# Tom-Ryder/VIforSDEs

Measured on AMD Instinct MI355X. Metric: sampled-paths/sec + ELBO-iters/sec (value = global_batch * ELBO-iters/s), higher is better.
Workload: dtype f32 (GRU/ELBO kernels) + bf16-autocast encoder; 1 GPU; lv: state_dim=2, T=400 (dt=0.1), batch=512/GPU, enc 256x8x4 heads, GRU 64x2; global_batch=512, parallelism=dp1, hip_graph=True

## Files before the change

### include/vsde_hip.h

```cpp
#ifndef VSDE_HIP_H
#define VSDE_HIP_H

#include <stddef.h>
#include <stdint.h>

#ifdef __cplusplus
extern "C" {
#endif

#define VSDE_ABI_VERSION 1

#define VSDE_E_BADARG (-1)
#define VSDE_E_LAYERS (-2)
#define VSDE_E_HIDDEN (-3)
#define VSDE_E_WORKSPACE (-4)
#define VSDE_E_STATE (-5)

#define VSDE_MAX_LAYERS 4
#define VSDE_MAX_HIDDEN 1024
#define VSDE_MAX_STATE 32

#define VSDE_CTX_F32 0
#define VSDE_CTX_BF16 1

// ... 83 lines not shown
                            int N, int C, int64_t mod_pitch, void *workspace, size_t workspace_bytes, void *stream);
int vsde_swiglu_fwd(int dtype, const void *u, void *out, int64_t M, int H2, void *stream);
int vsde_swiglu_bwd(int dtype, const void *u, const void *dout, void *du, int64_t M, int H2, void *stream);
int vsde_gate_merge_fwd(int dtype, const void *attn, const void *glog, void *out, int64_t B, int N, int heads, int d,
                        int token_major, int64_t glog_stride, void *stream);
int vsde_gate_merge_bwd(int dtype, const void *attn, const void *glog, const void *dout, void *dattn, void *dglog, int64_t B,
                        int N, int heads, int d, int token_major, int64_t glog_stride, void *stream);
int vsde_qk_norm_rope_fwd(int dtype, const void *qkv, const float *cosT, const float *sinT, const float *wq, const float *wk,
                          const void *v0, const float *lam, void *q, void *k, void *v, int64_t B, int N, int heads, int d,
                          double eps, int token_major, int64_t row_stride, void *stream);
int64_t vsde_qk_norm_rope_bwd_partials(int64_t B, int N, int heads, int d);
int vsde_qk_norm_rope_bwd(int dtype, const void *qkv, const float *cosT, const float *sinT, const float *wq, const float *wk,
                          const void *v0, const float *lam, const void *dq, const void *dk, const void *dv, void *dqkv,
                          void *dv0, float *dlam_partial, int64_t B, int N, int heads, int d, double eps, int token_major,
                          int64_t row_stride, int dv0_accumulate, const void *dv_extra, void *stream);

int vsde_attention_max_tokens(void);
int vsde_attention_fwd_bf16(const void *q, const void *k, const void *v, void *o, float *lse, int64_t B, int N, int H,
                            int head_dim, double scale, void *stream);
int vsde_attention_bwd_bf16(const void *dout, const void *q, const void *k, const void *v, const void *o, const float *lse,
                            void *dq, void *dk, void *dv, float *delta, int64_t B, int N, int H, int head_dim, double scale,
                            void *stream);

int vsde_attention_fused_supported(int N, int head_dim);
int vsde_attention_fwd_gated_bf16(const void *q, const void *k, const void *v, const void *gate, int64_t ldg, void *o, float *lse,
                                  int64_t B, int N, int H, double scale, void *stream);
int vsde_gate_bwd_delta(const void *dout, const void *og, const void *gate, int64_t ldg, void *dattn, void *dgate, int64_t ldd,
                        float *delta, int64_t B, int N, int H, void *stream);
int64_t vsde_attention_bwd_fused_partials(int64_t B, int N, int H);
int vsde_attention_bwd_fused_bf16(const void *dattn, const void *q, const void *k, const void *v, const float *lse, const float *delta,
                                  const float *rinv, const float *cosT, const float *sinT, const float *wq, const float *wk,
                                  const void *vdiff, const float *lam, void *dv0, int dv0_accumulate, const void *dv_extra, void *dy,
                                  int64_t ldy, float *dlam_partial, int64_t B, int N, int H, double scale, void *stream);

size_t vsde_linear_wgrad_workspace_bytes(int64_t M, int N, int K);
int vsde_linear_wgrad_bf16(const void *dy, const void *x, int64_t M, int N, int K, float *dW, float *db, void *workspace,
                           size_t workspace_bytes, void *stream);
int vsde_linear_wgrad_bf16_rows(const void *dy, const void *x, int64_t M, int N, int K, float *dW, float *db,
                                const int32_t *row_map, void *workspace, size_t workspace_bytes, void *stream);
typedef struct VsdeWgradItem {
    const void *dy, *x;
    int64_t M;
    int32_t N, K;
    float *dW, *db;
    const int32_t *row_map;
} VsdeWgradItem;
size_t vsde_linear_wgrad_group_workspace_bytes(int n, const void *items );
int vsde_linear_wgrad_group_bf16(int n, const void *items, int group_plan, void *workspace, size_t workspace_bytes, void *stream);

#define VSDE_EPI_PLAIN 0
#define VSDE_EPI_SWIGLU 1
#define VSDE_EPI_SWIGLU_BWD 2
int vsde_linear_bf16_supported(int64_t M, int N, int K, int epilogue);
int vsde_linear_bf16(const void *x, int64_t ldx, const void *w, const void *bias, void *y, int64_t ldy, int64_t M, int N, int K,
                     int epilogue, void *s_out, int64_t lds, const void *u_in, int64_t ldu, void *stream);
int vsde_linear_qknorm_bf16(const void *x, int64_t ldx, const void *w, const void *bias, int64_t M, int K, int heads, int gate_width,
                            int tokens, const float *cosT, const float *sinT, const float *wq, const float *wk, const void *v0,
                            const float *lam, double eps, void *q, void *k, void *v, void *gate, int64_t ldg, int gate_sigmoid,
                            float *rinv, void *vdiff, void *stream);
int vsde_linear_gated_bf16(const void *attn, int64_t ldx, const void *gate, int64_t ldgate, const void *w, const void *bias, void *y,
                           int64_t ldy, int64_t M, int N, int K, void *stream);

int vsde_linear_gate_bwd_bf16(const void *dy, int64_t ldy, const void *w_t, const void *og, const void *s, int64_t lds, void *dattn,
                              void *dgate, int64_t ldd, float *delta, int64_t M, int K, int heads, int tokens, void *stream);

int vsde_mlp_block_fwd_bf16(const void *x, const void *yin, const void *ga, const void *sc, const void *sh, const void *gm,
// ... 69 lines not shown
```

### viforsdes_amd/_hip.py

```python
from __future__ import annotations

import ctypes
import os
from typing import Optional, Sequence

import torch

from .build import LIB_PATH

VSDE_ABI_VERSION = 1
MAX_LAYERS = 4
MAX_HIDDEN = 1024
MAX_STATE = 32
DIAG_MIN = 1e-2


class HipLibraryError(RuntimeError):
    pass


class _Dims(ctypes.Structure):
    _fields_ = [(n, ctypes.c_int) for n in ("B", "T", "S", "P", "C", "H", "L")]


class _Weights(ctypes.Structure):
    _fields_ = [(n, ctypes.c_void_p) for n in (
        "W_ih_l0", "W_hh_l0", "b_ih_l0", "b_hh_l0", "W_ih_stack", "W_hh_stack",
        "b_ih_stack", "b_hh_stack", "out_weight", "out_bias")]


class _CtxView(ctypes.Structure):
    _fields_ = [("base", ctypes.c_void_p), ("dtype", ctypes.c_int),
                ("batch_stride", ctypes.c_int64), ("step_stride", ctypes.c_int64)]


class _Grads(ctypes.Structure):
    _fields_ = [(n, ctypes.c_void_p) for n in (
        "x0", "context", "theta", "W_ih_l0", "W_hh_l0", "b_ih_l0", "b_hh_l0",
        "W_ih_stack", "W_hh_stack", "b_ih_stack", "b_hh_stack", "out_weight", "out_bias")] + [
        ("context_dtype", ctypes.c_int), ("context_batch_stride", ctypes.c_int64)]


EXPORTS = (
    "vsde_abi_version", "vsde_build_ablations", "vsde_last_error",
    "vsde_head_forward_workspace_bytes", "vsde_head_forward",
    "vsde_head_backward_workspace_bytes", "vsde_head_backward",
    "vsde_elbo_path_terms", "vsde_elbo_path_terms_bwd", "vsde_elbo_tail_fwd", "vsde_elbo_tail_bwd",
    "vsde_log_weights", "vsde_log_weight_accumulate",
    "vsde_profile_enable", "vsde_profile_elapsed_ms", "vsde_debug_force_v1", "vsde_debug_head_mp", "vsde_head_mfma_range_exceeded",
    "vsde_ln_modulate_fwd", "vsde_ln_modulate_bwd", "vsde_gated_residual_fwd", "vsde_gated_residual_bwd",
    "vsde_swiglu_fwd", "vsde_swiglu_bwd", "vsde_gate_merge_fwd", "vsde_gate_merge_bwd",
    "vsde_qk_norm_rope_fwd", "vsde_qk_norm_rope_bwd_partials", "vsde_qk_norm_rope_bwd",
    "vsde_residual_ln_fwd", "vsde_residual_ln_bwd", "vsde_colsum_workspace_bytes", "vsde_linear_wgrad_workspace_bytes", "vsde_linear_wgrad_bf16", "vsde_linear_wgrad_bf16_rows", "vsde_linear_wgrad_group_workspace_bytes", "vsde_linear_wgrad_group_bf16",
    "vsde_attention_max_tokens", "vsde_attention_fwd_bf16", "vsde_attention_bwd_bf16",
    "vsde_attention_fused_supported", "vsde_attention_fwd_gated_bf16", "vsde_gate_bwd_delta", "vsde_attention_bwd_fused_partials",
    "vsde_attention_bwd_fused_bf16",
    "vsde_euler_maruyama_fwd", "vsde_euler_maruyama_bwd", "vsde_sde_coefficients_fwd", "vsde_sde_coefficients_bwd", "vsde_linear_bf16_supported", "vsde_linear_bf16", "vsde_linear_qknorm_bf16", "vsde_linear_gated_bf16", "vsde_linear_gate_bwd_bf16",
    "vsde_mlp_image_bytes", "vsde_mlp_fwd_bf16", "vsde_mlp_block_fwd_bf16", "vsde_mlp_attn_block_fwd_bf16", "vsde_linear_deep256_bf16", "vsde_mlp_debug_trace", "vsde_wgrad_debug_trace", "vsde_attn_debug_trace", "vsde_mlp_bwd_image_bytes", "vsde_mlp_bwd_bf16",
    "vsde_pack_tile_bytes", "vsde_pack_refresh", "vsde_optim_chunk_bytes", "vsde_optim_chunk_elems", "vsde_optim_step",
)

_lib: Optional[ctypes.CDLL] = None
_loaded_path: Optional[str] = None


def library_path() -> str:
    return _loaded_path or os.environ.get("VSDE_HIP_LIB") or LIB_PATH


def has_ablations() -> bool:
    return bool(load().vsde_build_ablations())


ABL_LIB_PATH = os.path.join(os.path.dirname(LIB_PATH), "libvsde_hip_abl.so")


def load() -> ctypes.CDLL:
    global _lib
    if _lib is not None:
        return _lib
    path = os.environ.get("VSDE_HIP_LIB") or LIB_PATH
    if not os.path.exists(path):
        raise HipLibraryError(
            f"{path} is missing: build it with `python -m viforsdes_amd.build` "
            "(there is no CPU fallback for the fused head / ELBO kernels)")
    lib = ctypes.CDLL(path)
    for name in EXPORTS:
        if not hasattr(lib, name):
            raise HipLibraryError(f"{path} does not export {name}")
    global _loaded_path
    _loaded_path = path
    lib.vsde_abi_version.restype = ctypes.c_int
    if lib.vsde_abi_version() != VSDE_ABI_VERSION:
        raise HipLibraryError(f"{path}: ABI version mismatch; rebuild it")
    lib.vsde_last_error.restype = ctypes.c_char_p
    lib.vsde_head_forward_workspace_bytes.restype = ctypes.c_size_t
    lib.vsde_head_backward_workspace_bytes.restype = ctypes.c_size_t
    for f in (lib.vsde_head_forward, lib.vsde_head_backward, lib.vsde_elbo_path_terms, lib.vsde_elbo_path_terms_bwd):
        f.restype = ctypes.c_int
    lib.vsde_qk_norm_rope_bwd_partials.restype = ctypes.c_int64
    lib.vsde_attention_bwd_fused_partials.restype = ctypes.c_int64
    lib.vsde_linear_wgrad_workspace_bytes.restype = ctypes.c_size_t
    lib.vsde_linear_wgrad_group_workspace_bytes.restype = ctypes.c_size_t
    lib.vsde_colsum_workspace_bytes.restype = ctypes.c_size_t
    lib.vsde_mlp_bwd_image_bytes.restype = ctypes.c_int64
    _lib = lib
    return lib


def _raise(rc: int) -> None:
    msg = load().vsde_last_error().decode("utf-8", "replace")
    if rc < 0:
        raise ValueError(msg)
    raise HipLibraryError(f"HIP error {rc}: {msg}")


def _ptr(t: Optional[torch.Tensor]):
    return ctypes.c_void_p(None if t is None or t.numel() == 0 else t.data_ptr())


def _require_hip(*tensors: torch.Tensor) -> torch.device:
    dev = None
    for t in tensors:
        if t is None:
            continue
        if not t.is_cuda:
            raise HipLibraryError(
                "the fused head / ELBO kernels only run on a HIP (cuda) device; got a "
                f"{t.device} tensor and there is no CPU fallback")
        if dev is None:
            dev = t.device
        elif t.device != dev:
            raise ValueError("all tensors must live on the same device")
    assert dev is not None
# ... 803 lines not shown
    du = torch.empty(M, 2 * H, device=dev, dtype=torch.bfloat16)
    dx = torch.empty(M, C, device=dev, dtype=torch.bfloat16)
    with torch.cuda.device(dev):
        _call(lib.vsde_mlp_bwd_bf16, _ptr(dy), _i64(lddy), _ptr(u), _i64(ldu), _ptr(img), _ptr(du), _i64(2 * H), _ptr(dx), _i64(C), _i64(M),
              ctypes.c_int(C), ctypes.c_int(H), _stream(dev))
    return du, dx


def linear_gate_bwd(dy: torch.Tensor, w_t: torch.Tensor, og: torch.Tensor, s: torch.Tensor, dgate: torch.Tensor, tokens: int):
    lib = load(); dev = _require_hip(dy, w_t, og, s, dgate)
    dy, ldy = _rows2d(dy); s, lds = _rows2d(s); dgate, ldd = _rows2d(dgate)
    B, N, H, d = og.shape
    M, K = dy.shape
    if d != 64 or N != tokens or M != B * N or tuple(w_t.shape) != (H * 64, K) or not (og.is_contiguous() and w_t.is_contiguous()):
        raise ValueError("linear_gate_bwd: inconsistent shapes")
    dattn = torch.empty_like(og)
    delta = torch.empty(B, H, N, device=dev, dtype=torch.float32)
    with torch.cuda.device(dev):
        _call(lib.vsde_linear_gate_bwd_bf16, _ptr(dy), _i64(ldy), _ptr(w_t), _ptr(og), _ptr(s), _i64(lds), _ptr(dattn), _ptr(dgate),
              _i64(ldd), _ptr(delta), _i64(M), ctypes.c_int(K), ctypes.c_int(H), ctypes.c_int(N), _stream(dev))
    return dattn, delta


def attention_bwd_fused(dattn, q, k, v, lse, delta, rinv, cos, sin, wq, wk, vdiff, lam, dv0, dv_extra, dy, scale: float):
    lib = load(); dev = _require_hip(dattn, q, k, v, lse, delta, rinv, dy)
    B, N, H, d = q.shape
    dy2, ldy = _rows2d(dy)
    accumulate = dv0 is not None
    parts = None
    if vdiff is not None:
        if dv0 is None:
            dv0 = torch.empty_like(v)
        parts = torch.empty(int(lib.vsde_attention_bwd_fused_partials(_i64(B), ctypes.c_int(N), ctypes.c_int(H))), device=dev, dtype=torch.float32)
    with torch.cuda.device(dev):
        _call(lib.vsde_attention_bwd_fused_bf16, _ptr(dattn), _ptr(q), _ptr(k), _ptr(v), _ptr(lse), _ptr(delta), _ptr(rinv), _ptr(cos),
              _ptr(sin), _ptr(wq), _ptr(wk), _ptr(vdiff), _ptr(lam if vdiff is not None else None),
              _ptr(dv0 if vdiff is not None else None), ctypes.c_int(int(accumulate)), _ptr(dv_extra), _ptr(dy2), _i64(ldy), _ptr(parts),
              _i64(B), ctypes.c_int(N), ctypes.c_int(H), ctypes.c_double(scale), _stream(dev))
    return (dv0 if vdiff is not None else None), (parts.sum() if parts is not None else None)


def linear_gated_bf16(attn: torch.Tensor, gate: torch.Tensor, w: torch.Tensor, bias: Optional[torch.Tensor]):
    lib = load(); dev = _require_hip(attn, gate, w)
    attn, ldx = _rows2d(attn); gate, ldg = _rows2d(gate)
    M, K = attn.shape
    N = w.shape[0]
    y = torch.empty(M, N, device=dev, dtype=torch.bfloat16)
    with torch.cuda.device(dev):
        _call(lib.vsde_linear_gated_bf16, _ptr(attn), _i64(ldx), _ptr(gate), _i64(ldg), _ptr(w), _ptr(bias), _ptr(y), _i64(N), _i64(M),
              ctypes.c_int(N), ctypes.c_int(K), _stream(dev))
    return y


def linear_swiglu_bwd_bf16(dy: torch.Tensor, w_t: torch.Tensor, u: torch.Tensor):
    lib = load(); dev = _require_hip(dy, w_t, u)
    dy, ldx = _rows2d(dy)
    M, K = dy.shape
    H = w_t.shape[0]
    du = torch.empty(M, 2 * H, device=dev, dtype=torch.bfloat16)
    with torch.cuda.device(dev):
        _call(lib.vsde_linear_bf16, _ptr(dy), _i64(ldx), _ptr(w_t), None, _ptr(du), _i64(2 * H), _i64(M), ctypes.c_int(H),
              ctypes.c_int(K), ctypes.c_int(EPI_SWIGLU_BWD), None, _i64(0), _ptr(u), _i64(u.stride(0)), _stream(dev))
    return du
```

### viforsdes_amd/csrc/vsde_attn.hip

```cpp
#include <stdlib.h>

#include "vsde_common.h"

namespace vsde {

typedef float f32x16 __attribute__((ext_vector_type(16)));
typedef short bf16x8 __attribute__((ext_vector_type(8)));
typedef short bf16x4 __attribute__((ext_vector_type(4)));
typedef __bf16 bf16v2 __attribute__((ext_vector_type(2)));
typedef float f32v2 __attribute__((ext_vector_type(2)));

constexpr int AT_D = 64;
constexpr int AT_KLD = 72;
constexpr int AT_MAXN = 544;

struct AttnParams {
    const uint16_t *q, *k, *v;
    uint16_t *o;
    float *lse;
    int N, H;
    int npad;
    int vld;
    float scale, scale_log2e;
    const uint16_t *gate;
// ... 592 lines not shown
            p.trace[wave * 8 + 7] = npairs_;
        }
    }
#undef VSDE_F8_STAMP
}
#endif


struct QkBwd {
    uint16_t *dy; int64_t ldy;
    const float *rinv;
    const float *cosT, *sinT;
    const float *wq, *wk;
    const float *lam;
    const uint16_t *vdiff;
    uint16_t *dv0; int dv0_accumulate;
    const uint16_t *dv_extra;
    float *dlam_partial;
    int dbg;
};

struct AttnBwdParams {
    const uint16_t *q, *k, *v, *o, *dout;
    const float *lse;
    float *delta;
    uint16_t *dq, *dk, *dv;
    int N, H, ntile;
    float scale, scale_log2e;
    QkBwd f;
    int park_off;
    int split_dq, split_dkv;
    int split_pitch_dq, split_pitch_dkv;
    int nragged;
};

__device__ __forceinline__ f32x16 tile_product(const uint16_t *arow, const bf16x8 (&bfrag)[4]) {
    f32x16 t = {0, 0, 0, 0, 0, 0, 0, 0, 0, 0, 0, 0, 0, 0, 0, 0};
#pragma unroll
    for (int ks = 0; ks < 4; ++ks) t = __builtin_amdgcn_mfma_f32_32x32x16_bf16(*(const bf16x8 *)(arow + ks * 16), bfrag[ks], t, 0, 0, 0);
    return t;
}

typedef short bf16x4s __attribute__((ext_vector_type(4)));
__device__ __forceinline__ uint2 lds_read_tr(const uint16_t *ptr) {
    bf16x4s r = __builtin_amdgcn_ds_read_tr16_b64_v4i16((__attribute__((address_space(3))) bf16x4s *)ptr);
    return *(uint2 *)&r;
}

__device__ __forceinline__ void accumulate_transposed(const uint16_t *tile, int lane, const bf16x8 &b0, const bf16x8 &b1,
                                                      f32x16 &acc0, f32x16 &acc1) {
    const int h2 = lane >> 5, m = lane & 15;
    const uint16_t *src = tile + (4 * h2 + (m >> 2)) * AT_KLD + ((lane >> 4) & 1) * 16 + (m & 3) * 4;
#pragma unroll
    for (int dt = 0; dt < 2; ++dt) {
        const uint2 a0 = lds_read_tr(src + dt * 32), a1 = lds_read_tr(src + dt * 32 + 8 * AT_KLD);
        const uint2 a2 = lds_read_tr(src + dt * 32 + 16 * AT_KLD), a3 = lds_read_tr(src + dt * 32 + 24 * AT_KLD);
        uint4 w0 = make_uint4(a0.x, a0.y, a1.x, a1.y), w1 = make_uint4(a2.x, a2.y, a3.x, a3.y);
        if (dt == 0) {
            acc0 = __builtin_amdgcn_mfma_f32_32x32x16_bf16(*(bf16x8 *)&w0, b0, acc0, 0, 0, 0);
            acc0 = __builtin_amdgcn_mfma_f32_32x32x16_bf16(*(bf16x8 *)&w1, b1, acc0, 0, 0, 0);
        } else {
            acc1 = __builtin_amdgcn_mfma_f32_32x32x16_bf16(*(bf16x8 *)&w0, b0, acc1, 0, 0, 0);
            acc1 = __builtin_amdgcn_mfma_f32_32x32x16_bf16(*(bf16x8 *)&w1, b1, acc1, 0, 0, 0);
        }
    }
}
// ... 833 lines not shown
            }
        }
    }
    if constexpr (!FUSED) {
#pragma unroll
        for (int blk = 0; blk < 2; ++blk) {
            const int query = (2 * wave + blk) * 32 + fr;
            if (qok[blk]) store_transposed(p.dq + base + query * ts, h2, acc[blk][0], acc[blk][1], p.scale);
        }
    } else {
        int lane_e = lane;
        asm volatile("" : "+v"(lane_e));
        NormRowsIn in[2];
#pragma unroll
        for (int blk = 0; blk < 2; ++blk)
            if ((2 * wave + blk) * 32 < N) norm_rinv_request<0>(p.f, in[blk], (int64_t)b * N, (2 * wave + blk) * 32, N, hh, p.H, lane_e);
        __syncthreads();
        float *slice = (float *)asmem + wave * AT_ESLICE;
#pragma unroll
        for (int blk = 0; blk < 2; ++blk) {
            const int tok0 = (2 * wave + blk) * 32;
            if (tok0 < N) {
                norm_rows_from_frags(in[blk], (uint16_t *)slice, qf[blk], lane_e);
                stage_acc_tile(slice, acc[blk][0], acc[blk][1], p.scale, lane_e);
                wave_lds_fence();
                staged_norm_rope_bwd<0>(p.f, slice, in[blk], (int64_t)b * N, tok0, N, hh, p.H, lane_e);
                wave_lds_fence();
            }
        }
    }
}
#endif

template <bool FUSED, bool ONE = false, int BT = AT_BT>
__global__ void __launch_bounds__(BT, AT_BT / BT) attn_bwd_dkv_kernel(AttnBwdParams p) {
    extern __shared__ __attribute__((aligned(16))) uint16_t asmem[];
    const int tid = threadIdx.x, lane = tid & 63, wave = tid >> 6, fr = lane & 31, h2 = lane >> 5;
    const int b = blockIdx.x / p.H, hh = blockIdx.x - b * p.H, N = p.N, npad = p.ntile * 32;
    uint16_t *Qs = asmem, *Os = asmem + npad * AT_KLD;
    float *lse2s = (float *)(asmem + 2 * npad * AT_KLD), *dels = lse2s + npad;
    const int64_t ts = (int64_t)p.H * AT_D, base = ((int64_t)b * N * p.H + hh) * AT_D;
    const int64_t srow = ((int64_t)b * p.H + hh) * N;
    bf16x8 kn[4], vn[4];
    auto request = [&](int kblk) {
        const int key = kblk * 32 + fr;
        const bool ok = kblk < p.ntile && key < N;
        load_bfrag(p.k + base, ts, key, ok, h2, kn);
        load_bfrag(p.v + base, ts, key, ok, h2, vn);
    };
    request(wave);
    constexpr int NWV = BT / 64;
    const bool split = FUSED && p.split_dkv != 0;
    const bool sharer = split && wave < 4;
    bf16x8 kx[4], vx[4];
    if constexpr (FUSED) {
        if (sharer) {
            const int key = NWV * 32 + fr;
            load_bfrag(p.k + base, ts, key, key < N, h2, kx);
            load_bfrag(p.v + base, ts, key, key < N, h2, vx);
        }
    }
    stage_two<BT, (BT == AT_BT ? AT_MAXN : AT_MAXN_SMALL)>(p.q + base, p.dout + base, ts, N, npad, tid, Qs, Os);
    for (int i = tid; i < npad; i += BT) {
        lse2s[i] = i < N ? p.lse[srow + i] * 1.4426950408889634f : INFINITY;
        dels[i] = i < N ? p.delta[srow + i] : 0.f;
    }
    __syncthreads();
    const float c2 = p.scale_log2e;
    f32x16 dk0, dk1, dv0, dv1;
    auto sweep = [&](const bf16x8 (&kf)[4], const bf16x8 (&vf)[4], int qt0, int qt1) {
#pragma unroll 1
        for (int qt = qt0; qt < qt1; ++qt) {
            const uint16_t *qt_ = Qs + qt * 32 * AT_KLD, *dot_ = Os + qt * 32 * AT_KLD;
            const f32x16 sc = tile_product(qt_ + fr * AT_KLD + h2 * 8, kf);
            const f32x16 dp = tile_product(dot_ + fr * AT_KLD + h2 * 8, vf);
            float pr[16], ds[16];
#pragma unroll
            for (int g = 0; g < 4; ++g) {
                const float4 l4 = *(const float4 *)(lse2s + qt * 32 + 8 * g + 4 * h2);
                const float4 d4 = *(const float4 *)(dels + qt * 32 + 8 * g + 4 * h2);
                const float lv[4] = {l4.x, l4.y, l4.z, l4.w}, dv[4] = {d4.x, d4.y, d4.z, d4.w};
#pragma unroll
                for (int e = 0; e < 4; ++e) {
                    const int r = 4 * g + e;
                    pr[r] = fast_exp2(fmaf(sc[r], c2, -lv[e]));
                    ds[r] = pr[r] * (dp[r] - dv[e]);
                }
            }
            bf16x8 p0, p1, s0, s1;
            pack_tile(pr, p0, p1);
            pack_tile(ds, s0, s1);
            accumulate_transposed(dot_, lane, p0, p1, dv0, dv1);
            accumulate_transposed(qt_, lane, s0, s1, dk0, dk1);
        }
    };
    if constexpr (FUSED) {
        if (sharer) {
            char *mine = (char *)asmem + p.split_dkv + wave * p.split_pitch_dkv;
            keep_frags((uint4 *)mine, kn, vn, lane);
            asm volatile("" : "+v"(mine));
#pragma unroll
            for (int e = 0; e < 16; ++e) { dk0[e] = 0.f; dk1[e] = 0.f; dv0[e] = 0.f; dv1[e] = 0.f; }
            sweep(kx, vx, (p.ntile * wave) >> 2, (p.ntile * (wave + 1)) >> 2);
            restore_frags((const uint4 *)mine, kn, vn, lane);
            asm volatile("" : "+v"(mine));
            const bool ok = NWV * 32 + fr < N;
            stage_acc_rows((float *)mine, dv0, dv1, 1.0f, lane, ok);
            stage_acc_rows((float *)mine + p.nragged * AT_ELD, dk0, dk1, p.scale, lane, ok);
        }
    }
    const int nblk = split ? NWV : p.ntile;
    int last = -1;
    int parked = -1;
    bf16x8 ykeep[4];
#pragma unroll
    for (int ks = 0; ks < 4; ++ks) ykeep[ks] = bf16x8{0, 0, 0, 0, 0, 0, 0, 0};
    for (int kblk = wave; kblk < nblk; kblk += NWV) {
        if (kblk != wave) request(kblk);
        const int key = kblk * 32 + fr;
        const bool kok = key < N;
        bf16x8 kf[4], vf[4];
#pragma unroll
        for (int ks = 0; ks < 4; ++ks) { kf[ks] = kn[ks]; vf[ks] = vn[ks]; }
#pragma unroll
        for (int e = 0; e < 16; ++e) { dk0[e] = 0.f; dk1[e] = 0.f; dv0[e] = 0.f; dv1[e] = 0.f; }
        sweep(kf, vf, 0, p.ntile);
        if constexpr (FUSED) {
            asm volatile("" ::: "memory");
            if constexpr (ONE) {
                last = kblk;
#pragma unroll
                for (int ks = 0; ks < 4; ++ks) ykeep[ks] = kf[ks];
                continue;
            }
            if (kblk + NWV >= nblk && !(p.f.dbg & 8)) { last = kblk; continue; }
            if (p.park_off != 0 && kblk < NWV && !(p.f.dbg & 8)) {
                float *park = (float *)((char *)asmem + p.park_off) + wave * (2 * AT_ESLICE);
                stage_acc_tile(park, dv0, dv1, 1.0f, lane);
                stage_acc_tile(park + AT_ESLICE, dk0, dk1, p.scale, lane);
                parked = kblk;
                continue;
            }
            const int64_t m = (int64_t)b * N + key;
            float dl = 0.f;
            if (p.f.dbg & 2) { if (kok) store_transposed(p.f.dy + m * p.f.ldy + (2 * p.H + hh) * 64, h2, dv0, dv1, 1.0f); }
            else dl = kok ? value_bwd_store(p.f, dv0, dv1, m, hh, p.H, lane) : 0.f;
            if (p.f.dlam_partial != nullptr) {
                dl = wave_sum(dl);
                if (lane == 0) p.f.dlam_partial[(int64_t)blockIdx.x * p.ntile + kblk] = dl;
            }
            if (p.f.dbg & 1) { if (kok) store_transposed(p.f.dy + m * p.f.ldy + (p.H + hh) * 64, h2, dk0, dk1, p.scale); }
            else norm_rope_bwd_store<1>(p.f, dk0, dk1, p.scale, kf, m, key, hh, p.H, lane, kok);
        } else if (kok) {
            store_transposed(p.dk + base + key * ts, h2, dk0, dk1, p.scale);
            store_transposed(p.dv + base + key * ts, h2, dv0, dv1, 1.0f);
        }
    }
    if constexpr (FUSED) {
        int lane_e = lane, wave_e = wave;
        asm volatile("" : "+v"(lane_e), "+v"(wave_e));
        const int64_t m0 = (int64_t)b * N;
        NormRowsIn kin; ValueRowsIn vin;
        if constexpr (!ONE) { if (p.f.dbg & 64) last = -1; }
        if (last >= 0) {
            value_rows_request(p.f, vin, m0, last * 32, N, hh, p.H, lane_e);
            if constexpr (ONE) norm_rinv_request<1>(p.f, kin, m0, last * 32, N, hh, p.H, lane_e);
            else norm_rows_request<1>(p.f, kin, p.k + base, ts, m0, last * 32, N, hh, p.H, lane_e);
        }
        if (split && wave_e == 4) value_rows_touch(p.f, m0, NWV * 32, N, hh, p.H, lane_e);
        if (split && wave_e == 5) norm_rows_touch<1>(p.f, p.k + base, ts, m0, NWV * 32, N, hh, p.H, lane_e);
        __syncthreads();
        if (last >= 0) {
            float *slice = (float *)asmem + wave_e * AT_ESLICE;
            const int vreps = (split && wave_e == 4) ? 2 : 1;
            stage_acc_tile(slice, dv0, dv1, 1.0f, lane_e);
#pragma unroll 1
            for (int rep = 0; rep < vreps; ++rep) {
                const int blk = rep == 0 ? last : NWV;
                if (rep != 0) {
                    value_rows_request(p.f, vin, m0, blk * 32, N, hh, p.H, lane_e);
                    sum_partial_tiles(slice, (const float *)((const char *)asmem + p.split_dkv), p.split_pitch_dkv / 4, p.nragged, lane_e);
                }
                wave_lds_fence();
                int lane_v = lane_e;
                asm volatile("" : "+v"(lane_v));
                float dl = (!ONE && (p.f.dbg & 32)) ? 0.f : staged_value_bwd(p.f, slice, vin, m0, blk * 32, N, hh, p.H, lane_v);
                if (p.f.dlam_partial != nullptr) {
                    dl = wave_sum(dl);
                    if (lane_e == 0) p.f.dlam_partial[(int64_t)blockIdx.x * p.ntile + blk] = dl;
                }
                wave_lds_fence();
            }
            int lane_k = lane_e;
            asm volatile("" : "+v"(lane_k));
            if constexpr (ONE) norm_rows_from_frags(kin, (uint16_t *)slice, ykeep, lane_k);
            stage_acc_tile(slice, dk0, dk1, p.scale, lane_k);
            wave_lds_fence();
            if (ONE || !(p.f.dbg & 16)) staged_norm_rope_bwd<1>(p.f, slice, kin, m0, last * 32, N, hh, p.H, lane_k);
            if (split && wave_e == 5) {
                norm_rows_request<1>(p.f, kin, p.k + base, ts, m0, NWV * 32, N, hh, p.H, lane_k);
                wave_lds_fence();
                sum_partial_tiles(slice, (const float *)((const char *)asmem + p.split_dkv) + p.nragged * AT_ELD, p.split_pitch_dkv / 4, p.nragged, lane_k);
                wave_lds_fence();
                staged_norm_rope_bwd<1>(p.f, slice, kin, m0, NWV * 32, N, hh, p.H, lane_k);
            }
        }
        if (!ONE && parked >= 0) {
            const float *park = (const float *)((char *)asmem + p.park_off) + wave_e * (2 * AT_ESLICE);
            value_rows_request(p.f, vin, m0, parked * 32, N, hh, p.H, lane_e);
            norm_rows_request<1>(p.f, kin, p.k + base, ts, m0, parked * 32, N, hh, p.H, lane_e);
            wave_lds_fence();
            float dl = staged_value_bwd(p.f, park, vin, m0, parked * 32, N, hh, p.H, lane_e);
            if (p.f.dlam_partial != nullptr) {
                dl = wave_sum(dl);
                if (lane_e == 0) p.f.dlam_partial[(int64_t)blockIdx.x * p.ntile + parked] = dl;
            }
            staged_norm_rope_bwd<1>(p.f, park + AT_ESLICE, kin, m0, parked * 32, N, hh, p.H, lane_e);
        }
    }
}

__global__ void __launch_bounds__(256) gate_bwd_delta_kernel(const uint16_t *__restrict__ dout, const uint16_t *__restrict__ og,
                                                             const uint16_t *__restrict__ gate, int64_t ldg, uint16_t *__restrict__ dattn,
                                                             uint16_t *__restrict__ dgate, int64_t ldd, float *__restrict__ delta,
                                                             int64_t M, int N, int H) {
    const int64_t gid = (int64_t)blockIdx.x * blockDim.x + threadIdx.x;
    const bool ok = gid < M * 8;
    const int64_t m = ok ? gid >> 3 : M - 1;
    const int k = (int)(gid & 7) * 8;
    const int64_t b = m / N, n = m - b * N;
    const uint4 g4 = *(const uint4 *)(gate + m * ldg + k);
    const uint32_t gw[4] = {g4.x, g4.y, g4.z, g4.w};
    float s[8], acc[8];
#pragma unroll
    for (int e = 0; e < 4; ++e) { s[2 * e] = bfl(gw[e]); s[2 * e + 1] = bfh(gw[e]); }
#pragma unroll
    for (int e = 0; e < 8; ++e) acc[e] = 0.f;
    for (int hh = 0; hh < H; ++hh) {
        const int64_t off = (m * H + hh) * 64 + k;
        const uint4 d4 = *(const uint4 *)(dout + off), o4 = *(const uint4 *)(og + off);
        const uint32_t dw[4] = {d4.x, d4.y, d4.z, d4.w}, ow[4] = {o4.x, o4.y, o4.z, o4.w};
        uint32_t r[4];
        float dsum = 0.f;
#pragma unroll
        for (int e = 0; e < 4; ++e) {
            const float d0 = bfl(dw[e]), d1 = bfh(dw[e]), p0 = d0 * bfl(ow[e]), p1 = d1 * bfh(ow[e]);
            acc[2 * e] += p0; acc[2 * e + 1] += p1; dsum += p0 + p1;
            r[e] = pack_bf16(d0 * s[2 * e], d1 * s[2 * e + 1]);
        }
        dsum += __shfl_xor(dsum, 1, 64); dsum += __shfl_xor(dsum, 2, 64); dsum += __shfl_xor(dsum, 4, 64);
        if (ok) {
// ... 160 lines not shown

extern "C" int vsde_attention_fused_supported(int N, int head_dim) { return head_dim == AT_D && N > 0 && N <= AT_MAXN && !force_stream(); }

extern "C" int vsde_attention_fwd_gated_bf16(const void *q, const void *k, const void *v, const void *gate, int64_t ldg, void *o,
                                             float *lse, int64_t B, int N, int H, double scale, void *stream) {
    VSDE_CHECK_ARG(q && k && v && gate && o && lse && B > 0 && N > 0 && H > 0, VSDE_E_BADARG, "bad gated attention arguments");
    VSDE_CHECK_ARG(vsde_attention_fused_supported(N, AT_D), VSDE_E_BADARG, "gated attention runs the LDS-resident kernel: N <= %d", AT_MAXN);
    VSDE_CHECK_ARG(ldg >= 64 && ldg % 4 == 0 && ((uintptr_t)gate % 8) == 0 && B * H < (1LL << 31), VSDE_E_BADARG, "bad gate rows");
    AttnParams p;
    p.q = (const uint16_t *)q; p.k = (const uint16_t *)k; p.v = (const uint16_t *)v; p.o = (uint16_t *)o; p.lse = lse;
    p.N = N; p.H = H; p.npad = (N + 31) & ~31; p.vld = p.npad + 4;
    p.scale = (float)scale; p.scale_log2e = (float)(scale * 1.4426950408889634);
    p.gate = (const uint16_t *)gate; p.ldg = ldg;
    const size_t lds = (size_t)2 * p.npad * AT_KLD * sizeof(uint16_t);
    return launch_attn_fwd(p, B * H, lds, (hipStream_t)stream);
}

extern "C" int vsde_gate_bwd_delta(const void *dout, const void *og, const void *gate, int64_t ldg, void *dattn, void *dgate, int64_t ldd,
                                   float *delta, int64_t B, int N, int H, void *stream) {
    VSDE_CHECK_ARG(dout && og && gate && dattn && dgate && delta && B > 0 && N > 0 && H > 0, VSDE_E_BADARG, "bad gate_bwd_delta arguments");
    VSDE_CHECK_ARG(ldg >= 64 && ldg % 8 == 0 && ldd >= 64 && ldd % 8 == 0 && ((uintptr_t)gate % 16) == 0 && ((uintptr_t)dgate % 16) == 0 &&
                   ((uintptr_t)dout % 16) == 0 && ((uintptr_t)og % 16) == 0 && ((uintptr_t)dattn % 16) == 0, VSDE_E_BADARG,
                   "gate_bwd_delta operands must be 16-byte aligned with row pitches that are multiples of 8 elements");
    const int64_t M = B * N, blocks = (M * 8 + 255) / 256;
    VSDE_CHECK_ARG(blocks < (1LL << 31), VSDE_E_BADARG, "too many rows");
    hipLaunchKernelGGL(gate_bwd_delta_kernel, dim3((unsigned)blocks), dim3(256), 0, (hipStream_t)stream, (const uint16_t *)dout,
                       (const uint16_t *)og, (const uint16_t *)gate, ldg, (uint16_t *)dattn, (uint16_t *)dgate, ldd, delta, M, N, H);
    VSDE_CHECK_HIP(hipGetLastError());
    return 0;
}

extern "C" int64_t vsde_attention_bwd_fused_partials(int64_t B, int N, int H) { return B * H * ((N + 31) / 32); }

extern "C" int vsde_attention_bwd_fused_bf16(const void *dattn, const void *q, const void *k, const void *v, const float *lse,
                                             const float *delta, const float *rinv, const float *cosT, const float *sinT,
                                             const float *wq, const float *wk, const void *vdiff, const float *lam, void *dv0,
                                             int dv0_accumulate, const void *dv_extra, void *dy, int64_t ldy, float *dlam_partial,
                                             int64_t B, int N, int H, double scale, void *stream) {
    VSDE_CHECK_ARG(dattn && q && k && v && lse && delta && rinv && cosT && sinT && wq && wk && dy && B > 0 && N > 0 && H > 0, VSDE_E_BADARG,
                   "bad attention_bwd_fused arguments");
    VSDE_CHECK_ARG(vsde_attention_fused_supported(N, AT_D), VSDE_E_BADARG, "attention_bwd_fused runs the LDS-resident kernels: N <= %d", AT_MAXN);
    VSDE_CHECK_ARG((!vdiff) == (!lam) && (!vdiff) == (!dv0) && (!vdiff) == (!dlam_partial), VSDE_E_BADARG,
                   "value mixing needs vdiff, lam, dv0 and dlam_partial together");
    VSDE_CHECK_ARG(ldy >= 3 * H * 64 && ldy % 4 == 0 && ((uintptr_t)dy % 8) == 0 && ((uintptr_t)cosT % 16) == 0 && ((uintptr_t)sinT % 16) == 0 &&
                   ((uintptr_t)wq % 16) == 0 && ((uintptr_t)wk % 16) == 0 && B * H < (1LL << 31), VSDE_E_BADARG, "bad attention_bwd_fused buffers");
    AttnBwdParams p = {};
    p.q = (const uint16_t *)q; p.k = (const uint16_t *)k; p.v = (const uint16_t *)v; p.o = nullptr;
    p.dout = (const uint16_t *)dattn; p.lse = lse; p.delta = (float *)delta;
    p.N = N; p.H = H; p.ntile = (N + 31) / 32;
    p.scale = (float)scale; p.scale_log2e = (float)(scale * 1.4426950408889634);
    p.f.dy = (uint16_t *)dy; p.f.ldy = ldy; p.f.rinv = rinv; p.f.cosT = cosT; p.f.sinT = sinT; p.f.wq = wq; p.f.wk = wk; p.f.lam = lam;
    p.f.vdiff = (const uint16_t *)vdiff; p.f.dv0 = (uint16_t *)dv0; p.f.dv0_accumulate = dv0_accumulate;
    p.f.dv_extra = (const uint16_t *)dv_extra; p.f.dlam_partial = dlam_partial;
    { static int dbg = -1; if (dbg < 0) dbg = ablation_env("VSDE_ATTN_DEBUG"); p.f.dbg = dbg; }
    const size_t stage = (size_t)(AT_BT / 64) * AT_ESLICE * sizeof(float);
    size_t lds_dq = (size_t)2 * p.ntile * 32 * AT_KLD * sizeof(uint16_t), lds_dkv = lds_dq + (size_t)2 * p.ntile * 32 * sizeof(float);
    lds_dq = lds_dq > stage ? lds_dq : stage; lds_dkv = lds_dkv > stage ? lds_dkv : stage;
    {
        const int waves = AT_BT / 64, two_round = p.ntile > waves ? p.ntile - waves : 0;
        const size_t park = (size_t)two_round * 2 * AT_ESLICE * sizeof(float);
        if (two_round > 0 && p.ntile <= 2 * waves && lds_dkv + park <= 160 * 1024) { p.park_off = (int)lds_dkv; lds_dkv += park; }
    }
    {
        static int on = -1;
        if (on < 0) on = (int)vsde_knob("VSDE_ATTN_SPLIT", 1);
        const int waves = AT_BT / 64;
        if (on && p.f.dbg == 0 && p.ntile == waves + 1) {
            p.nragged = N - waves * 32;
            const size_t tile = (size_t)p.nragged * AT_ELD * sizeof(float), keep = 8 * 64 * 16;
            const size_t pitch_dq = tile > keep ? tile : keep, pitch_dkv = 2 * tile > keep ? 2 * tile : keep;
            if (lds_dq + 4 * pitch_dq <= 160 * 1024) { p.split_dq = (int)lds_dq; p.split_pitch_dq = (int)pitch_dq; lds_dq += 4 * pitch_dq; }
            const size_t operands = lds_dkv - (p.park_off ? (size_t)2 * AT_ESLICE * sizeof(float) : 0);
            if (operands + 4 * pitch_dkv <= 160 * 1024) {
                p.split_dkv = (int)operands; p.split_pitch_dkv = (int)pitch_dkv; p.park_off = 0; lds_dkv = operands + 4 * pitch_dkv;
            }
        }
    }
    hipStream_t s = (hipStream_t)stream;
    const int nwv = AT_BT / 64;
    if (p.f.dbg == 0 && small_wg_enabled() && p.ntile <= AT_BT_SMALL / 64) {
        const size_t stage_s = (size_t)(AT_BT_SMALL / 64) * AT_ESLICE * sizeof(float);
        size_t l_dq = (size_t)2 * p.ntile * 32 * AT_KLD * sizeof(uint16_t), l_dkv = l_dq + (size_t)2 * p.ntile * 32 * sizeof(float);
        l_dq = l_dq > stage_s ? l_dq : stage_s; l_dkv = l_dkv > stage_s ? l_dkv : stage_s;
        p.park_off = 0; p.split_dq = 0; p.split_dkv = 0;
        VSDE_CHECK_HIP(hipFuncSetAttribute((const void *)attn_bwd_dq_kernel<true, true, AT_BT_SMALL>, hipFuncAttributeMaxDynamicSharedMemorySize, (int)l_dq));
        VSDE_CHECK_HIP(hipFuncSetAttribute((const void *)attn_bwd_dkv_kernel<true, true, AT_BT_SMALL>, hipFuncAttributeMaxDynamicSharedMemorySize, (int)l_dkv));
        hipLaunchKernelGGL((attn_bwd_dq_kernel<true, true, AT_BT_SMALL>), dim3((unsigned)(B * H)), dim3(AT_BT_SMALL), l_dq, s, p);
        hipLaunchKernelGGL((attn_bwd_dkv_kernel<true, true, AT_BT_SMALL>), dim3((unsigned)(B * H)), dim3(AT_BT_SMALL), l_dkv, s, p);
        VSDE_CHECK_HIP(hipGetLastError());
        return 0;
    }
#ifdef VSDE_ABLATIONS
    if (p.f.dbg == 0 && dq_wide_enabled() && p.ntile > 4 && p.ntile <= 16) {
        VSDE_CHECK_HIP(hipFuncSetAttribute((const void *)attn_bwd_dq_wide_kernel<true>, hipFuncAttributeMaxDynamicSharedMemorySize, (int)lds_dq));
        hipLaunchKernelGGL(attn_bwd_dq_wide_kernel<true>, dim3((unsigned)(B * H)), dim3(512), lds_dq, s, p);
    } else
#endif
    if (p.f.dbg == 0 && (p.ntile <= nwv || p.split_dq != 0)) {
        VSDE_CHECK_HIP(hipFuncSetAttribute((const void *)attn_bwd_dq_kernel<true, true>, hipFuncAttributeMaxDynamicSharedMemorySize, (int)lds_dq));
        hipLaunchKernelGGL((attn_bwd_dq_kernel<true, true>), dim3((unsigned)(B * H)), dim3(AT_BT), lds_dq, s, p);
    } else {
        VSDE_CHECK_HIP(hipFuncSetAttribute((const void *)attn_bwd_dq_kernel<true>, hipFuncAttributeMaxDynamicSharedMemorySize, (int)lds_dq));
        hipLaunchKernelGGL(attn_bwd_dq_kernel<true>, dim3((unsigned)(B * H)), dim3(AT_BT), lds_dq, s, p);
    }
    if (p.f.dbg == 0 && (p.ntile <= nwv || p.split_dkv != 0)) {
        VSDE_CHECK_HIP(hipFuncSetAttribute((const void *)attn_bwd_dkv_kernel<true, true>, hipFuncAttributeMaxDynamicSharedMemorySize, (int)lds_dkv));
        hipLaunchKernelGGL((attn_bwd_dkv_kernel<true, true>), dim3((unsigned)(B * H)), dim3(AT_BT), lds_dkv, s, p);
    } else {
        VSDE_CHECK_HIP(hipFuncSetAttribute((const void *)attn_bwd_dkv_kernel<true>, hipFuncAttributeMaxDynamicSharedMemorySize, (int)lds_dkv));
        hipLaunchKernelGGL(attn_bwd_dkv_kernel<true>, dim3((unsigned)(B * H)), dim3(AT_BT), lds_dkv, s, p);
    }
    VSDE_CHECK_HIP(hipGetLastError());
    return 0;
}
```

Baseline: 19750 paths/s.

## Store dS from dK/dV kernel and compute dQ from it in chunks

The fused attention backward now has the dK/dV kernel write each bf16 dS tile to a global workspace. A new dQ kernel reads those tiles back and multiplies them by K, instead of recomputing QK^T, the softmax and dP. Pairs are processed in chunks of up to 256 so the workspace stays bounded. This trades recomputation for extra global writes and reads, plus more kernel launches per chunk, and it falls back to the old path when the small-workgroup variant applies.

```diff
diff --git a/include/vsde_hip.h b/include/vsde_hip.h
--- a/include/vsde_hip.h
+++ b/include/vsde_hip.h
@@ -139,6 +139,12 @@
                                   const float *rinv, const float *cosT, const float *sinT, const float *wq, const float *wk,
                                   const void *vdiff, const float *lam, void *dv0, int dv0_accumulate, const void *dv_extra, void *dy,
                                   int64_t ldy, float *dlam_partial, int64_t B, int N, int H, double scale, void *stream);
+int64_t vsde_attention_bwd_fused_ds_bytes(int64_t B, int N, int H);
+int vsde_attention_bwd_fused_ds_bf16(const void *dattn, const void *q, const void *k, const void *v, const float *lse,
+                                     const float *delta, const float *rinv, const float *cosT, const float *sinT, const float *wq,
+                                     const float *wk, const void *vdiff, const float *lam, void *dv0, int dv0_accumulate,
+                                     const void *dv_extra, void *dy, int64_t ldy, float *dlam_partial, int64_t B, int N, int H,
+                                     double scale, void *ds, int64_t ds_bytes, void *stream);
 
 size_t vsde_linear_wgrad_workspace_bytes(int64_t M, int N, int K);
 int vsde_linear_wgrad_bf16(const void *dy, const void *x, int64_t M, int N, int K, float *dW, float *db, void *workspace,
diff --git a/viforsdes_amd/_hip.py b/viforsdes_amd/_hip.py
--- a/viforsdes_amd/_hip.py
+++ b/viforsdes_amd/_hip.py
@@ -54,7 +54,7 @@
     "vsde_residual_ln_fwd", "vsde_residual_ln_bwd", "vsde_colsum_workspace_bytes", "vsde_linear_wgrad_workspace_bytes", "vsde_linear_wgrad_bf16", "vsde_linear_wgrad_bf16_rows", "vsde_linear_wgrad_group_workspace_bytes", "vsde_linear_wgrad_group_bf16",
     "vsde_attention_max_tokens", "vsde_attention_fwd_bf16", "vsde_attention_bwd_bf16",
     "vsde_attention_fused_supported", "vsde_attention_fwd_gated_bf16", "vsde_gate_bwd_delta", "vsde_attention_bwd_fused_partials",
-    "vsde_attention_bwd_fused_bf16",
+    "vsde_attention_bwd_fused_bf16", "vsde_attention_bwd_fused_ds_bytes", "vsde_attention_bwd_fused_ds_bf16",
     "vsde_euler_maruyama_fwd", "vsde_euler_maruyama_bwd", "vsde_sde_coefficients_fwd", "vsde_sde_coefficients_bwd", "vsde_linear_bf16_supported", "vsde_linear_bf16", "vsde_linear_qknorm_bf16", "vsde_linear_gated_bf16", "vsde_linear_gate_bwd_bf16",
     "vsde_mlp_image_bytes", "vsde_mlp_fwd_bf16", "vsde_mlp_block_fwd_bf16", "vsde_mlp_attn_block_fwd_bf16", "vsde_linear_deep256_bf16", "vsde_mlp_debug_trace", "vsde_wgrad_debug_trace", "vsde_attn_debug_trace", "vsde_mlp_bwd_image_bytes", "vsde_mlp_bwd_bf16",
     "vsde_pack_tile_bytes", "vsde_pack_refresh", "vsde_optim_chunk_bytes", "vsde_optim_chunk_elems", "vsde_optim_step",
@@ -100,6 +100,7 @@
         f.restype = ctypes.c_int
     lib.vsde_qk_norm_rope_bwd_partials.restype = ctypes.c_int64
     lib.vsde_attention_bwd_fused_partials.restype = ctypes.c_int64
+    lib.vsde_attention_bwd_fused_ds_bytes.restype = ctypes.c_int64
     lib.vsde_linear_wgrad_workspace_bytes.restype = ctypes.c_size_t
     lib.vsde_linear_wgrad_group_workspace_bytes.restype = ctypes.c_size_t
     lib.vsde_colsum_workspace_bytes.restype = ctypes.c_size_t
@@ -969,11 +970,13 @@
         if dv0 is None:
             dv0 = torch.empty_like(v)
         parts = torch.empty(int(lib.vsde_attention_bwd_fused_partials(_i64(B), ctypes.c_int(N), ctypes.c_int(H))), device=dev, dtype=torch.float32)
-    with torch.cuda.device(dev):
-        _call(lib.vsde_attention_bwd_fused_bf16, _ptr(dattn), _ptr(q), _ptr(k), _ptr(v), _ptr(lse), _ptr(delta), _ptr(rinv), _ptr(cos),
+    ds_bytes = int(lib.vsde_attention_bwd_fused_ds_bytes(_i64(B), ctypes.c_int(N), ctypes.c_int(H)))
+    ds = torch.empty(ds_bytes, device=dev, dtype=torch.uint8) if ds_bytes > 0 else None
+    with torch.cuda.device(dev):
+        _call(lib.vsde_attention_bwd_fused_ds_bf16, _ptr(dattn), _ptr(q), _ptr(k), _ptr(v), _ptr(lse), _ptr(delta), _ptr(rinv), _ptr(cos),
               _ptr(sin), _ptr(wq), _ptr(wk), _ptr(vdiff), _ptr(lam if vdiff is not None else None),
               _ptr(dv0 if vdiff is not None else None), ctypes.c_int(int(accumulate)), _ptr(dv_extra), _ptr(dy2), _i64(ldy), _ptr(parts),
-              _i64(B), ctypes.c_int(N), ctypes.c_int(H), ctypes.c_double(scale), _stream(dev))
+              _i64(B), ctypes.c_int(N), ctypes.c_int(H), ctypes.c_double(scale), _ptr(ds), _i64(ds_bytes), _stream(dev))
     return (dv0 if vdiff is not None else None), (parts.sum() if parts is not None else None)
 
 
diff --git a/viforsdes_amd/csrc/vsde_attn.hip b/viforsdes_amd/csrc/vsde_attn.hip
--- a/viforsdes_amd/csrc/vsde_attn.hip
+++ b/viforsdes_amd/csrc/vsde_attn.hip
@@ -648,6 +648,8 @@
     int split_dq, split_dkv;
     int split_pitch_dq, split_pitch_dkv;
     int nragged;
+    uint16_t *ds;
+    int pair0;
 };
 
 __device__ __forceinline__ f32x16 tile_product(const uint16_t *arow, const bf16x8 (&bfrag)[4]) {
@@ -1547,11 +1549,12 @@
 }
 #endif
 
-template <bool FUSED, bool ONE = false, int BT = AT_BT>
+template <bool FUSED, bool ONE = false, int BT = AT_BT, bool DS = false>
 __global__ void __launch_bounds__(BT, AT_BT / BT) attn_bwd_dkv_kernel(AttnBwdParams p) {
     extern __shared__ __attribute__((aligned(16))) uint16_t asmem[];
     const int tid = threadIdx.x, lane = tid & 63, wave = tid >> 6, fr = lane & 31, h2 = lane >> 5;
-    const int b = blockIdx.x / p.H, hh = blockIdx.x - b * p.H, N = p.N, npad = p.ntile * 32;
+    const int pair = DS ? (int)blockIdx.x + p.pair0 : (int)blockIdx.x;
+    const int b = pair / p.H, hh = pair - b * p.H, N = p.N, npad = p.ntile * 32;
     uint16_t *Qs = asmem, *Os = asmem + npad * AT_KLD;
     float *lse2s = (float *)(asmem + 2 * npad * AT_KLD), *dels = lse2s + npad;
     const int64_t ts = (int64_t)p.H * AT_D, base = ((int64_t)b * N * p.H + hh) * AT_D;
@@ -1583,7 +1586,9 @@
     __syncthreads();
     const float c2 = p.scale_log2e;
     f32x16 dk0, dk1, dv0, dv1;
-    auto sweep = [&](const bf16x8 (&kf)[4], const bf16x8 (&vf)[4], int qt0, int qt1) {
+    auto sweep = [&](const bf16x8 (&kf)[4], const bf16x8 (&vf)[4], int qt0, int qt1, int kblk) {
+        uint16_t *dsb = nullptr;
+        if constexpr (DS) dsb = p.ds + ((int64_t)blockIdx.x * p.ntile + __builtin_amdgcn_readfirstlane(kblk)) * p.ntile * 1024;
 #pragma unroll 1
         for (int qt = qt0; qt < qt1; ++qt) {
             const uint16_t *qt_ = Qs + qt * 32 * AT_KLD, *dot_ = Os + qt * 32 * AT_KLD;
@@ -1605,6 +1610,11 @@
             bf16x8 p0, p1, s0, s1;
             pack_tile(pr, p0, p1);
             pack_tile(ds, s0, s1);
+            if constexpr (DS) {
+                const uint32_t o = (uint32_t)qt * 2048u + (uint32_t)lane * 16u;
+                *(bf16x8 *)((char *)dsb + o) = s0;
+                *(bf16x8 *)((char *)dsb + o + 1024u) = s1;
+            }
             accumulate_transposed(dot_, lane, p0, p1, dv0, dv1);
             accumulate_transposed(qt_, lane, s0, s1, dk0, dk1);
         }
@@ -1616,7 +1626,7 @@
             asm volatile("" : "+v"(mine));
 #pragma unroll
             for (int e = 0; e < 16; ++e) { dk0[e] = 0.f; dk1[e] = 0.f; dv0[e] = 0.f; dv1[e] = 0.f; }
-            sweep(kx, vx, (p.ntile * wave) >> 2, (p.ntile * (wave + 1)) >> 2);
+            sweep(kx, vx, (p.ntile * wave) >> 2, (p.ntile * (wave + 1)) >> 2, NWV);
             restore_frags((const uint4 *)mine, kn, vn, lane);
             asm volatile("" : "+v"(mine));
             const bool ok = NWV * 32 + fr < N;
@@ -1639,7 +1649,7 @@
         for (int ks = 0; ks < 4; ++ks) { kf[ks] = kn[ks]; vf[ks] = vn[ks]; }
 #pragma unroll
         for (int e = 0; e < 16; ++e) { dk0[e] = 0.f; dk1[e] = 0.f; dv0[e] = 0.f; dv1[e] = 0.f; }
-        sweep(kf, vf, 0, p.ntile);
+        sweep(kf, vf, 0, p.ntile, kblk);
         if constexpr (FUSED) {
             asm volatile("" ::: "memory");
             if constexpr (ONE) {
@@ -1662,7 +1672,7 @@
             else dl = kok ? value_bwd_store(p.f, dv0, dv1, m, hh, p.H, lane) : 0.f;
             if (p.f.dlam_partial != nullptr) {
                 dl = wave_sum(dl);
-                if (lane == 0) p.f.dlam_partial[(int64_t)blockIdx.x * p.ntile + kblk] = dl;
+                if (lane == 0) p.f.dlam_partial[(int64_t)pair * p.ntile + kblk] = dl;
             }
             if (p.f.dbg & 1) { if (kok) store_transposed(p.f.dy + m * p.f.ldy + (p.H + hh) * 64, h2, dk0, dk1, p.scale); }
             else norm_rope_bwd_store<1>(p.f, dk0, dk1, p.scale, kf, m, key, hh, p.H, lane, kok);
@@ -1702,7 +1712,7 @@
                 float dl = (!ONE && (p.f.dbg & 32)) ? 0.f : staged_value_bwd(p.f, slice, vin, m0, blk * 32, N, hh, p.H, lane_v);
                 if (p.f.dlam_partial != nullptr) {
                     dl = wave_sum(dl);
-                    if (lane_e == 0) p.f.dlam_partial[(int64_t)blockIdx.x * p.ntile + blk] = dl;
+                    if (lane_e == 0) p.f.dlam_partial[(int64_t)pair * p.ntile + blk] = dl;
                 }
                 wave_lds_fence();
             }
@@ -1728,10 +1738,89 @@
             float dl = staged_value_bwd(p.f, park, vin, m0, parked * 32, N, hh, p.H, lane_e);
             if (p.f.dlam_partial != nullptr) {
                 dl = wave_sum(dl);
-                if (lane_e == 0) p.f.dlam_partial[(int64_t)blockIdx.x * p.ntile + parked] = dl;
+                if (lane_e == 0) p.f.dlam_partial[(int64_t)pair * p.ntile + parked] = dl;
             }
             staged_norm_rope_bwd<1>(p.f, park + AT_ESLICE, kin, m0, parked * 32, N, hh, p.H, lane_e);
         }
+    }
+}
+
+constexpr int DQ_BT = 512, DQ_PF = 4, DQ_SLICE = 32 * 32;
+
+__device__ __forceinline__ int dq_slot(int row, int granule) { return row * 32 + 4 * (granule ^ ((row >> 1) & 7)); }
+
+__global__ void __launch_bounds__(DQ_BT, 4) attn_bwd_dq_from_ds_kernel(AttnBwdParams p) {
+    extern __shared__ __attribute__((aligned(16))) uint16_t asmem[];
+    const int tid = threadIdx.x, lane = tid & 63, wave = tid >> 6, fr = lane & 31, h2 = lane >> 5;
+    const int pair = (int)blockIdx.x + p.pair0;
+    const int b = pair / p.H, hh = pair - b * p.H, N = p.N, ntile = p.ntile, npad = ntile * 32;
+    uint16_t *Ks = asmem, *Ts = asmem + npad * AT_KLD + wave * DQ_SLICE;
+    const int64_t ts = (int64_t)p.H * AT_D, base = ((int64_t)b * N * p.H + hh) * AT_D;
+    constexpr int NW = DQ_BT / 64;
+    uint4 pf[DQ_PF][2];
+    const char *dsp = (const char *)(p.ds + (int64_t)blockIdx.x * ntile * ntile * 1024);
+    auto load_tile = [&](int qblk, int kblk, uint4 (&x)[2]) {
+        const uint32_t o = (uint32_t)(kblk * ntile + qblk) * 2048u + (uint32_t)lane * 16u;
+        x[0] = *(const uint4 *)(dsp + o); x[1] = *(const uint4 *)(dsp + o + 1024u);
+    };
+    auto issue = [&](int qblk) {
+#pragma unroll
+        for (int u = 0; u < DQ_PF; ++u) load_tile(qblk, min(u, ntile - 1), pf[u]);
+    };
+    if (wave < ntile) issue(wave);
+    {
+        constexpr int SIT = (AT_MAXN * 8 + DQ_BT - 1) / DQ_BT;
+        uint4 r[SIT];
+#pragma unroll
+        for (int it = 0; it < SIT; ++it) {
+            const int i = tid + it * DQ_BT, n = i >> 3, c = i & 7;
+            r[it] = (i < npad * 8 && n < N) ? *(const uint4 *)(p.k + base + n * ts + c * 8) : make_uint4(0, 0, 0, 0);
+        }
+#pragma unroll
+        for (int it = 0; it < SIT; ++it) {
+            const int i = tid + it * DQ_BT, n = i >> 3, c = i & 7;
+            if (i < npad * 8) *(uint4 *)(Ks + n * AT_KLD + c * 8) = r[it];
+        }
+    }
+    __syncthreads();
+    const int m = lane & 15, rr = 4 * h2 + (m >> 2), gr = 4 * ((lane >> 4) & 1) + (m & 3);
+    const int rd0 = dq_slot(rr, gr), rd1 = dq_slot(rr + 8, gr), rd2 = dq_slot(rr + 16, gr), rd3 = dq_slot(rr + 24, gr);
+    for (int qblk = wave; qblk < ntile; qblk += NW) {
+        const int query = qblk * 32 + fr;
+        const bool qok = query < N;
+        f32x16 acc0, acc1;
+#pragma unroll
+        for (int e = 0; e < 16; ++e) { acc0[e] = 0.f; acc1[e] = 0.f; }
+        auto consume = [&](const uint4 (&x)[2], int kblk) {
+            *(uint2 *)(Ts + dq_slot(fr, h2)) = make_uint2(x[0].x, x[0].y);
+            *(uint2 *)(Ts + dq_slot(fr, 2 + h2)) = make_uint2(x[0].z, x[0].w);
+            *(uint2 *)(Ts + dq_slot(fr, 4 + h2)) = make_uint2(x[1].x, x[1].y);
+            *(uint2 *)(Ts + dq_slot(fr, 6 + h2)) = make_uint2(x[1].z, x[1].w);
+            wave_lds_fence();
+            const uint2 a0 = lds_read_tr(Ts + rd0), a1 = lds_read_tr(Ts + rd1), a2 = lds_read_tr(Ts + rd2), a3 = lds_read_tr(Ts + rd3);
+            uint4 w0 = make_uint4(a0.x, a0.y, a1.x, a1.y), w1 = make_uint4(a2.x, a2.y, a3.x, a3.y);
+            accumulate_transposed(Ks + kblk * 32 * AT_KLD, lane, *(bf16x8 *)&w0, *(bf16x8 *)&w1, acc0, acc1);
+            wave_lds_fence();
+        };
+#pragma unroll 1
+        for (int k0 = 0; k0 < ntile; k0 += DQ_PF) {
+#pragma unroll
+            for (int u = 0; u < DQ_PF; ++u) {
+                const int kblk = k0 + u;
+                if (kblk < ntile) consume(pf[u], kblk);
+                if (u == DQ_PF / 2 - 1 || u == DQ_PF - 1) {
+#pragma unroll
+                    for (int v = u + 1 - DQ_PF / 2; v <= u; ++v)
+                        load_tile(qblk, min(k0 + v + DQ_PF, ntile - 1), pf[v]);
+                }
+            }
+        }
+        int lane_e = lane, query_e = query;
+        asm volatile("" : "+v"(lane_e), "+v"(query_e));
+        bf16x8 qf[4];
+        load_bfrag(p.q + base, ts, query_e, qok, lane_e >> 5, qf);
+        norm_rope_bwd_store<0>(p.f, acc0, acc1, p.scale, qf, (int64_t)b * N + query_e, query_e, hh, p.H, lane_e, qok);
+        if (qblk + NW < ntile) issue(qblk + NW);
     }
 }
 
@@ -1958,11 +2047,23 @@
 
 extern "C" int64_t vsde_attention_bwd_fused_partials(int64_t B, int N, int H) { return B * H * ((N + 31) / 32); }
 
-extern "C" int vsde_attention_bwd_fused_bf16(const void *dattn, const void *q, const void *k, const void *v, const float *lse,
-                                             const float *delta, const float *rinv, const float *cosT, const float *sinT,
-                                             const float *wq, const float *wk, const void *vdiff, const float *lam, void *dv0,
-                                             int dv0_accumulate, const void *dv_extra, void *dy, int64_t ldy, float *dlam_partial,
-                                             int64_t B, int N, int H, double scale, void *stream) {
+static int64_t ds_pair_bytes(int N) {
+    const int64_t ntile = (N + 31) / 32;
+    return (small_wg_enabled() && ntile <= AT_BT_SMALL / 64) ? 0 : ntile * ntile * 1024 * (int64_t)sizeof(uint16_t);
+}
+
+static int64_t ds_chunk_pairs(int64_t pairs) { return pairs < 256 ? pairs : 256; }
+
+extern "C" int64_t vsde_attention_bwd_fused_ds_bytes(int64_t B, int N, int H) {
+    if (B <= 0 || N <= 0 || H <= 0 || !vsde_attention_fused_supported(N, AT_D)) return 0;
+    return ds_chunk_pairs(B * H) * ds_pair_bytes(N);
+}
+
+static int attention_bwd_fused(const void *dattn, const void *q, const void *k, const void *v, const float *lse,
+                               const float *delta, const float *rinv, const float *cosT, const float *sinT,
+                               const float *wq, const float *wk, const void *vdiff, const float *lam, void *dv0,
+                               int dv0_accumulate, const void *dv_extra, void *dy, int64_t ldy, float *dlam_partial,
+                               int64_t B, int N, int H, double scale, void *ds, int64_t ds_bytes, void *stream) {
     VSDE_CHECK_ARG(dattn && q && k && v && lse && delta && rinv && cosT && sinT && wq && wk && dy && B > 0 && N > 0 && H > 0, VSDE_E_BADARG,
                    "bad attention_bwd_fused arguments");
     VSDE_CHECK_ARG(vsde_attention_fused_supported(N, AT_D), VSDE_E_BADARG, "attention_bwd_fused runs the LDS-resident kernels: N <= %d", AT_MAXN);
@@ -2016,6 +2117,29 @@
         VSDE_CHECK_HIP(hipGetLastError());
         return 0;
     }
+    if (ds != nullptr) {
+        const int64_t per = ds_pair_bytes(N), pairs = B * H;
+        VSDE_CHECK_ARG(((uintptr_t)ds % 16) == 0 && ds_bytes >= per, VSDE_E_BADARG, "the dS workspace holds no pair (%lld bytes each)",
+                       (long long)per);
+        const int64_t chunk = ds_bytes / per;
+        const size_t lds_q = (size_t)p.ntile * 32 * AT_KLD * sizeof(uint16_t) + (size_t)(DQ_BT / 64) * DQ_SLICE * sizeof(uint16_t);
+        const void *dkv = (p.f.dbg == 0 && (p.ntile <= nwv || p.split_dkv != 0)) ? (const void *)attn_bwd_dkv_kernel<true, true, AT_BT, true>
+                                                                                 : (const void *)attn_bwd_dkv_kernel<true, false, AT_BT, true>;
+        VSDE_CHECK_HIP(hipFuncSetAttribute(dkv, hipFuncAttributeMaxDynamicSharedMemorySize, (int)lds_dkv));
+        VSDE_CHECK_HIP(hipFuncSetAttribute((const void *)attn_bwd_dq_from_ds_kernel, hipFuncAttributeMaxDynamicSharedMemorySize, (int)lds_q));
+        p.ds = (uint16_t *)ds;
+        for (int64_t c0 = 0; c0 < pairs; c0 += chunk) {
+            const int64_t n = pairs - c0 < chunk ? pairs - c0 : chunk;
+            p.pair0 = (int)c0;
+            if (dkv == (const void *)attn_bwd_dkv_kernel<true, true, AT_BT, true>)
+                hipLaunchKernelGGL((attn_bwd_dkv_kernel<true, true, AT_BT, true>), dim3((unsigned)n), dim3(AT_BT), lds_dkv, s, p);
+            else
+                hipLaunchKernelGGL((attn_bwd_dkv_kernel<true, false, AT_BT, true>), dim3((unsigned)n), dim3(AT_BT), lds_dkv, s, p);
+            hipLaunchKernelGGL(attn_bwd_dq_from_ds_kernel, dim3((unsigned)n), dim3(DQ_BT), lds_q, s, p);
+        }
+        VSDE_CHECK_HIP(hipGetLastError());
+        return 0;
+    }
 #ifdef VSDE_ABLATIONS
     if (p.f.dbg == 0 && dq_wide_enabled() && p.ntile > 4 && p.ntile <= 16) {
         VSDE_CHECK_HIP(hipFuncSetAttribute((const void *)attn_bwd_dq_wide_kernel<true>, hipFuncAttributeMaxDynamicSharedMemorySize, (int)lds_dq));
@@ -2039,3 +2163,23 @@
     VSDE_CHECK_HIP(hipGetLastError());
     return 0;
 }
+
+extern "C" int vsde_attention_bwd_fused_bf16(const void *dattn, const void *q, const void *k, const void *v, const float *lse,
+                                             const float *delta, const float *rinv, const float *cosT, const float *sinT,
+                                             const float *wq, const float *wk, const void *vdiff, const float *lam, void *dv0,
+                                             int dv0_accumulate, const void *dv_extra, void *dy, int64_t ldy, float *dlam_partial,
+                                             int64_t B, int N, int H, double scale, void *stream) {
+    return attention_bwd_fused(dattn, q, k, v, lse, delta, rinv, cosT, sinT, wq, wk, vdiff, lam, dv0, dv0_accumulate, dv_extra, dy, ldy,
+                               dlam_partial, B, N, H, scale, nullptr, 0, stream);
+}
+
+extern "C" int vsde_attention_bwd_fused_ds_bf16(const void *dattn, const void *q, const void *k, const void *v, const float *lse,
+                                                const float *delta, const float *rinv, const float *cosT, const float *sinT,
+                                                const float *wq, const float *wk, const void *vdiff, const float *lam, void *dv0,
+                                                int dv0_accumulate, const void *dv_extra, void *dy, int64_t ldy, float *dlam_partial,
+                                                int64_t B, int N, int H, double scale, void *ds, int64_t ds_bytes, void *stream) {
+    if (N > 0 && ds_pair_bytes(N) == 0) ds = nullptr;
+    else VSDE_CHECK_ARG(ds != nullptr, VSDE_E_BADARG, "attention_bwd_fused_ds needs the dS workspace (vsde_attention_bwd_fused_ds_bytes)");
+    return attention_bwd_fused(dattn, q, k, v, lse, delta, rinv, cosT, sinT, wq, wk, vdiff, lam, dv0, dv0_accumulate, dv_extra, dy, ldy,
+                               dlam_partial, B, N, H, scale, ds, ds_bytes, stream);
+}
```

Result: slower. 19040 paths/s, median of 2 (-3.6%).
